# matteocarnelos/microflow-rs

Hardware: AMD Instinct MI355X
Metric: inferences/sec (int8) for person_detect.tflite (higher is better)
Workload: dtype i8; 1 GPU; person_detect.tflite batch=65536 per GPU, predict_inner int8->int8, inputs resident in HBM; per_gpu_batch=65536, global_batch=65536, parallelism=batch shard x1, no data-path collective

## Files before the change

### microflow_rs_amd/csrc/fused.hip

```cpp
#include <algorithm>
#include <cmath>
#include <cstdio>
#include <cstring>
#include <memory>

#include "ops_impl.hpp"
#include "wimage.hpp"

namespace mf {

struct FusedImpl {
    enum Kind { DWPW, TAIL, FCSM, STAGE, DWFC, PAIRTAIL, QUAD, CHAIN, FCCHAIN, POOLFC, PAIRBAND, PAIRWZ } kind;
    OpImpl *a, *b, *c;
    k::DwPwArgs dwpw;
    k::TailArgs tail;
    std::string name;
    k::StageArgs stage{};
    int stage_pairs = 0;
    std::vector<std::unique_ptr<DevBuf>> stage_w;
    k::DwFcArgs dwfc{};
    k::PairTailArgs pairtail{};
    k::PairFrontArgs pairfront{};
    bool has_front = false;
    k::QuadArgs quad{};
// ... 577 lines not shown
    if (magic != t.magic) return nullptr;
    std::unique_ptr<FusedImpl> f(new FusedImpl{FusedImpl::PAIRTAIL, dw, pairtail->b, pairtail->c, {}, {}, "pair_front_tail<6,6,128,2,256|3,3,256,2>"});
    f->pairtail = t, f->has_front = true, f->epi_mode = magic;
    k::PairFrontArgs &a = f->pairfront;
    a.dw_wmm = df.wmm, a.dwA = df.A, a.dwS = df.S, a.dwK = magic ? kc_with_magic(*f, dw->h_Kc) : df.Kc;
    a.dw_lo = df.lo_f, a.dw_hi = df.hi_f, a.izp4 = df.izp4;
    a.pw_w = plain_pw_image(*f, pw);
    a.pwA = pw->conv.A, a.pwS = pw->conv.S, a.pwK = magic ? kc_with_magic(*f, pw->h_Kc) : pw->conv.Kc;
    a.pw_lo = pw->conv.lo_f, a.pw_hi = pw->conv.hi_f;
    return f.release();
}

static FusedImpl *quad_group(FusedImpl *p1, FusedImpl *p2, const k::DwPwArgs &a, const k::DwPwArgs &b, const char *name, bool mm) {
    const OpSpec &d1 = p1->a->s, &q1 = p1->b->s, &d2 = p2->a->s, &q2 = p2->b->s;
    FusedImpl *f = new FusedImpl{FusedImpl::QUAD, p1->a, p2->b, nullptr, {}, {}, name};
    f->quad.a = a, f->quad.b = b, f->quad_mm = mm;
    f->epi_mode = std::min(pair_mode(a), pair_mode(b));
    f->quad_ops[0] = p1->a, f->quad_ops[1] = p1->b, f->quad_ops[2] = p2->a, f->quad_ops[3] = p2->b;
    const int shp[10] = {d1.H, d1.W, d1.C, d1.sh, q1.N, d2.H, d2.W, d2.C, d2.sh, q2.N};
    for (int i = 0; i < 10; ++i) f->quad_shape[i] = shp[i];
    return f;
}
FusedImpl *fused_quad_create(FusedImpl *p1, FusedImpl *p2) {
    const bool off = switches().no_quad;
    if (off || !p1 || !p2 || p1->kind != FusedImpl::DWPW || p2->kind != FusedImpl::DWPW) return nullptr;
    const OpSpec &d1 = p1->a->s, &q1 = p1->b->s, &d2 = p2->a->s, &q2 = p2->b->s;
    if (p1->a->device != p2->a->device || d1.u8 != d2.u8) return nullptr;
    if (d2.H != q1.H || d2.W != q1.W || d2.C != q1.N) return nullptr;
    if (k::quad_mm_shape(d1.H, d1.W, d1.C, d1.sh, q1.N, d2.H, d2.W, d2.C, d2.sh, q2.N)) {
        if (switches().no_quad_mm) return nullptr;
        k::DwPwArgs a = p1->dwpw, b = p2->dwpw;
        if (pair_mode(a) != 3 || pair_mode(b) != 3) a = pair_args(p1->a, p1->b, 0), b = pair_args(p2->a, p2->b, 0);
        if (!a.dw.wmm || !a.pw.wprep || !b.dw.wmm || !b.pw.wprep) return nullptr;
        if (!a.dw.magic || !a.pw.magic || !b.dw.magic || !b.pw.magic) return nullptr;
        return quad_group(p1, p2, a, b, "quad_mm<12,12,64,1,64|12,12,64,2,128>", true);
    }
    const char *nm = k::quad_name(d1.H, d1.W, d1.C, d1.sh, q1.N, d2.H, d2.W, d2.C, d2.sh, q2.N);
    if (!nm) return nullptr;
    const bool fma = p1->a->fma_strict() && p1->b->fma_strict() && p2->a->fma_strict() && p2->b->fma_strict();
    const k::DwPwArgs a = pair_args(p1->a, p1->b, fma ? 1 : 0), b = pair_args(p2->a, p2->b, fma ? 1 : 0);
    if (!a.dw.wmm || !a.pw.wrr || !b.dw.wmm || !b.pw.wrr) return nullptr;
    if (!a.dw.magic || !a.pw.magic || !b.dw.magic || !b.pw.magic) return nullptr;
    return quad_group(p1, p2, a, b, nm, false);
}

FusedImpl *fused_quad_stem_create(OpImpl *stem, FusedImpl *quad) {
    const bool off = switches().no_penta;
    if (off || !stem || !quad || quad->kind != FusedImpl::QUAD || quad->quad.stem || stem->fast != OpImpl::DW_STEM) return nullptr;
    const OpSpec &t = stem->s, &d1 = quad->a->s;
    if (stem->device != quad->a->device || t.u8 != d1.u8 || stem->force_generic) return nullptr;
    if (t.OH != d1.H || t.OW != d1.W || t.N != d1.C || t.sh != 2 || t.sw != 2 || t.C != 1) return nullptr;
    const int *q = quad->quad_shape;
    const char *nm = k::quad_stem_name(t.H, t.W, q[0], q[1], q[2], q[3], q[4], q[5], q[6], q[7], q[8], q[9]);
    if (!nm || !stem->stem.magic) return nullptr;
    std::unique_ptr<FusedImpl> f(new FusedImpl{FusedImpl::QUAD, stem, quad->b, nullptr, {}, {}, nm});
    f->quad = quad->quad;
    for (int i = 0; i < 10; ++i) f->quad_shape[i] = q[i];
    OpImpl *const *qo = quad->quad_ops;
    const bool fma = stem->fma_strict() && qo[0]->fma_strict() && qo[1]->fma_strict() && qo[2]->fma_strict() && qo[3]->fma_strict();
    f->quad.a = pair_args(qo[0], qo[1], fma ? 1 : 0), f->quad.b = pair_args(qo[2], qo[3], fma ? 1 : 0);
    k::DwStemArgs sa = stem->stem;
    if (fma) sa.use_fma();
    std::vector<uint32_t> tab(152);
    for (int l = 0; l < 64; ++l) tab[(size_t)2 * l] = sa.wmm[l][0], tab[(size_t)2 * l + 1] = sa.wmm[l][1];
    for (int c = 0; c < 8; ++c) {
        memcpy(&tab[(size_t)128 + c], &sa.A[c], 4);
// ... 414 lines not shown
```

### microflow_rs_amd/csrc/k_common.hpp

```cpp
#pragma once
#include <hip/hip_runtime.h>
#include <stdint.h>
#include <stdio.h>
#include <stdlib.h>

#include <atomic>
#include <type_traits>

#include "kernels.hpp"
#include "mf_switches.hpp"

namespace mf {
namespace k {

typedef int v4i __attribute__((ext_vector_type(4)));
typedef unsigned int u32x4 __attribute__((ext_vector_type(4)));

#ifndef MF_JITTER_DIAG
#define MF_JITTER_DIAG 0
#endif
__device__ __forceinline__ void mf_jitter() {
#if MF_JITTER_DIAG
    uint32_t t = (uint32_t)__builtin_readcyclecounter();
    t = (t ^ (t >> 7) ^ (threadIdx.x >> 6) * 0x9E3779B1u) * 0x85EBCA6Bu;
// ... 16 lines not shown
__device__ __forceinline__ int requant(int acc, float A, float S, float lo_f, float hi_f) {
    const float x = __fadd_rn(A, __fmul_rn(S, (float)acc));
    float r = __fadd_rn(x, __builtin_copysignf(0x1.fffffep-2f, x));
    r = __builtin_amdgcn_fmed3f(r, lo_f, hi_f);
    return (int)r;
}

template <int MG>
__device__ __forceinline__ int requant_t(int acc, float A, float S, float lo_f, float hi_f) {
    static_assert(MG != 3, "the single-fma form exists for the packed epilogues only (requant_pack4)");
    if constexpr (MG == 0) {
        return requant(acc, A, S, lo_f, hi_f);
    } else {
        const float f = __fsub_rn(__int_as_float(acc), 12582912.0f);
        const float x = __fadd_rn(A, __fmul_rn(S, f));
        float r = __fadd_rn(x, __builtin_copysignf(0x1.fffffep-2f, x));
        r = __builtin_amdgcn_fmed3f(r, lo_f, hi_f);
        return (int)r;
    }
}
template <int MG> __device__ __forceinline__ void epi_enter() {
    if constexpr (MG == 3) __builtin_amdgcn_s_setreg(0x801 , 3u );
}
#ifndef MF_EPI_PATCH_KO
#define MF_EPI_PATCH_KO 0
#endif
__device__ __forceinline__ EpiPatchRec epi_patch_load(const EpiPatchRec *tab, int idx) {
    typedef __attribute__((address_space(4))) const EpiPatchRec c_rec;
    if (MF_EPI_PATCH_KO || !tab) return EpiPatchRec{0, 0};
    c_rec *t = (c_rec *)(uintptr_t)tab;
    if (MF_EPI_PATCH_KO == 2) return EpiPatchRec{t[idx].P & 0, t[idx].meta};
    return EpiPatchRec{t[idx].P, t[idx].meta};
}
__device__ __forceinline__ void epi_patch_apply(v4i &a, const EpiPatchRec &rec, int g) {
    if (MF_EPI_PATCH_KO) return;
    if (__builtin_expect(rec.P != 0, 0)) {
        const bool any = (a[0] == rec.P) | (a[1] == rec.P) | (a[2] == rec.P) | (a[3] == rec.P);
        if (__builtin_expect(__builtin_amdgcn_ballot_w64(any) != 0ull, 0)) {
            asm volatile("" ::: "memory");
            const bool grp = g == ((rec.meta >> 2) & 3);
            const int delta = (rec.meta & 16) ? -1 : 1, reg = rec.meta & 3;
            a[0] += (grp && a[0] == rec.P) ? (reg == 0 ? delta : 0) : 0;
            a[1] += (grp && a[1] == rec.P) ? (reg == 1 ? delta : 0) : 0;
            a[2] += (grp && a[2] == rec.P) ? (reg == 2 ? delta : 0) : 0;
            a[3] += (grp && a[3] == rec.P) ? (reg == 3 ? delta : 0) : 0;
        }
    }
}
template <int MG> __device__ __forceinline__ int4 magic4(int4 k) {
    if constexpr (MG != 0) k.x += MF_MAGIC_I, k.y += MF_MAGIC_I, k.z += MF_MAGIC_I, k.w += MF_MAGIC_I;
    return k;
}

__device__ __forceinline__ int requant_any(int acc, float A, float S, float lo_f, float hi_f) {
    const float x = __fadd_rn(A, __fmul_rn(S, (float)acc));
    float r = __fadd_rn(x, __builtin_copysignf(0x1.fffffep-2f, x));
    r = (r != r) ? 0.0f : r;
    r = __builtin_amdgcn_fmed3f(r, lo_f, hi_f);
    return (int)r;
}

#ifndef MF_NT_STORE
#define MF_NT_STORE 0
#endif
template <bool NT> __device__ __forceinline__ void st_out_t(void *p, uint4 v) {
    if constexpr (NT) __builtin_nontemporal_store(v4i{(int)v.x, (int)v.y, (int)v.z, (int)v.w}, (v4i *)p);
    else *(v4i *)p = v4i{(int)v.x, (int)v.y, (int)v.z, (int)v.w};
}
template <bool NT> __device__ __forceinline__ void st_out_t(void *p, uint2 v) {
    typedef int v2i_ __attribute__((ext_vector_type(2)));
    if constexpr (NT) __builtin_nontemporal_store(v2i_{(int)v.x, (int)v.y}, (v2i_ *)p);
    else *(v2i_ *)p = v2i_{(int)v.x, (int)v.y};
}
template <bool NT> __device__ __forceinline__ void st_out_t(void *p, uint32_t v) {
    if constexpr (NT) __builtin_nontemporal_store(v, (uint32_t *)p);
    else *(uint32_t *)p = v;
}
template <typename V> __device__ __forceinline__ void st_out(void *p, V v) { st_out_t<MF_NT_STORE != 0>(p, v); }

__device__ __forceinline__ uint32_t pack4(int a, int b, int c, int d) {
// ... 264 lines not shown
        forced = now.dq_cfg;
        const char *l = now.dq_cfgs.c_str();
        if (*l) {
            int n = 1;
            for (const char *q = l; *q; ++q) n += *q == ',';
            int k = (int)(launches % (unsigned long)n);
            const char *q = l;
            while (k > 0 && *q) k -= *q++ == ',';
            forced = (int)strtol(q, nullptr, 0);
        }
    }
    if (forced) return forced;
    const double t_step = est_us * grid / (nsteps > 0 ? nsteps : 1);
    const int K = t_step >= 8.0 ? 1 : (t_step >= 4.0 ? 2 : 4);
    const double draws_per_us = nsteps / (K * (est_us > 1.0 ? est_us : 1.0));
    const double sfrac = sw.dq_static;
    int S0 = (int)(sfrac * (double)nsteps / (grid > 0 ? grid : 1));
    S0 = S0 < 2 ? 2 : (S0 > 32767 ? 32767 : S0);
    const int cfg = K | (draws_per_us > 60.0 ? 8 : 1) << 8 | S0 << 16;
    if (sw.dq_verbose) fprintf(stderr, "[microflow_amd] step queue: %d steps on %d workgroups, est %.0f us -> cfg 0x%x\n", nsteps, grid, est_us, cfg);
    return cfg;
}
static inline int *dq_slot(int *ring, unsigned long *launches) {
    if (!ring) return nullptr;
    const unsigned long n = launches ? __atomic_fetch_add(launches, 1ul, __ATOMIC_RELAXED) : dq_next_launch();
    return ring + (size_t)(n % (unsigned long)DYNQ_RING) * DynSteps::INTS;
}
static inline double dq_est_us(double hbm_bytes, double requant_bytes) {
    const double a = hbm_bytes / 4.5e6, b = requant_bytes / 4.0e6;
    return a > b ? a : b;
}

constexpr int cgcd(int a, int b) { return b == 0 ? a : cgcd(b, a % b); }
template <int TS> __device__ __forceinline__ constexpr int tile_swz(int x) {
    int r = 0;
    if constexpr ((TS & 0xf) != 0) r |= ((x >> ((TS & 0xf) - 1)) & 1);
    if constexpr (((TS >> 4) & 0xf) != 0) r |= ((x >> (((TS >> 4) & 0xf) - 1)) & 1) << 1;
    if constexpr (((TS >> 8) & 0xf) != 0) r |= ((x >> (((TS >> 8) & 0xf) - 1)) & 1) << 2;
    return r;
}

__device__ __forceinline__ float quant_div(float x, float scale, float rcp, bool fast) {
    if (!fast) return __fdiv_rn(x, scale);
    const float q0 = __fmul_rn(x, rcp);
    float q = __fmaf_rn(__fmaf_rn(-scale, q0, x), rcp, q0);
    if (!(__builtin_fabsf(q) <= 3.0e38f)) q = __fdiv_rn(x, scale);
    return q;
}

__device__ __forceinline__ void lane_group_transpose4(uint32_t &r0, uint32_t &r1, uint32_t &r2, uint32_t &r3) {
    typedef unsigned int u32x2 __attribute__((ext_vector_type(2)));
    u32x2 t;
    t = __builtin_amdgcn_permlane32_swap(r0, r2, false, false), r0 = t[0], r2 = t[1];
    t = __builtin_amdgcn_permlane32_swap(r1, r3, false, false), r1 = t[0], r3 = t[1];
    t = __builtin_amdgcn_permlane16_swap(r0, r1, false, false), r0 = t[0], r1 = t[1];
    t = __builtin_amdgcn_permlane16_swap(r2, r3, false, false), r2 = t[0], r3 = t[1];
}

struct LaunchState {
    static constexpr int MAX_DEV = 64;
    std::atomic<int> per_cu[MAX_DEV];
};
template <typename Kern> static int prepared(LaunchState &st, Kern kern, int threads, int lds_bytes) {
    int dev = 0;
    if (hipGetDevice(&dev) != hipSuccess || dev < 0 || dev >= LaunchState::MAX_DEV) dev = LaunchState::MAX_DEV - 1;
    int n = st.per_cu[dev].load(std::memory_order_relaxed);
// ... 40 lines not shown
```

### microflow_rs_amd/csrc/k_quad_mm.hip

```cpp
#include "k_common.hpp"

#ifndef MF_QMM_UB
#define MF_QMM_UB 2
#endif
#ifndef MF_QMM_KO
#define MF_QMM_KO 0
#endif
namespace mf {
namespace k {

namespace {
struct Q64 {
    static constexpr int G = 2, NTHR = 512, NWAVE = 8, NQ = 4, LP = 64, ROWB = 768;
    static constexpr int ROW_A = LP + ROWB + LP + 16, TILE_A = 14 * ROW_A, BUF_A = G * TILE_A;
    static constexpr int OPIX_A = 144, NPIX_A = G * OPIX_A, PLANE_A = NPIX_A * 16 + 16;
    static constexpr int ROW_B = LP + ROWB + LP, TILE_B = 14 * ROW_B, BUF_B = G * TILE_B, TS_B = 0x043;
    static constexpr int OPIX_B = 36, NPIX_B = G * OPIX_B, P16_B = 80, PLANE_B = P16_B * 16 + 16;
    static constexpr int OFF_TA = 0;
    static constexpr int OFF_MA = OFF_TA + BUF_A + 512;
    static constexpr int OFF_TB = OFF_MA + NQ * PLANE_A + 64;
    static constexpr int OFF_MB = OFF_TB + BUF_B + 512;
    static constexpr int OFF_C = OFF_MB + NQ * PLANE_B + 64;
    static constexpr int C_A_DW = 0, C_A_PW = 64 * 12, C_B_DW = 2 * 64 * 12, C_B_PW = 3 * 64 * 12, C_BYTES = 3 * 64 * 12 + 128 * 12;
    static constexpr int OFF_Q = OFF_C + C_BYTES;
    static constexpr int LDS = OFF_Q + 16;
};
static_assert(2 * Q64::LDS <= 160 * 1024, "two workgroups per CU");
static_assert(Q64::OFF_MA % 16 == 0 && Q64::OFF_TB % 16 == 0 && Q64::OFF_MB % 16 == 0, "16-byte aligned regions");
}

template <int MG, uint32_t XR4>
__global__ __launch_bounds__(512, 4) void quad_mm_12x12x64(const int8_t *__restrict__ in, int8_t *__restrict__ out, QuadArgs p, int batch) {
    using Z = Q64;
    constexpr int UB = MF_QMM_UB;
    epi_enter<MG>();
    extern __shared__ __attribute__((aligned(16))) uint8_t lds[];
    const int tid = threadIdx.x, lane = tid & 63;
    const int wave = __builtin_amdgcn_readfirstlane(tid >> 6);
    DynSteps dq;
    dq.init(lds + Z::OFF_Q, p.a.dw.queue, tid, p.a.dw.qcfg);

    for (int i = tid; i < (Z::BUF_A + 512) / 16; i += Z::NTHR)
        ((uint4 *)(lds + Z::OFF_TA))[i] = make_uint4(p.a.dw.izp4, p.a.dw.izp4, p.a.dw.izp4, p.a.dw.izp4);
    for (int i = tid; i < (Z::BUF_B + 512) / 16; i += Z::NTHR)
        ((uint4 *)(lds + Z::OFF_TB))[i] = make_uint4(p.b.dw.izp4, p.b.dw.izp4, p.b.dw.izp4, p.b.dw.izp4);

    const int col = lane & 15, g = lane >> 4;
    const int qa = wave & 3, ha = wave >> 2;
    const int cyA = col & 3, cxA = col >> 2;
    const int tbA = Z::OFF_TA + ha * Z::TILE_A + cyA * Z::ROW_A + Z::LP + (cxA + g - 1) * 64 + 16 * qa;
    const int mbA = Z::OFF_MA + qa * Z::PLANE_A + (ha * Z::OPIX_A + cyA * 12 + cxA) * 16 + 4 * g;
    const int cxB = col & 7, cyB = col >> 3;
    const int xlB = cxB * 2 + g - 1;
    const int tbB = Z::OFF_TB + ha * Z::TILE_B + cyB * 2 * Z::ROW_B + Z::LP + xlB * 64 + 16 * (qa ^ tile_swz<Z::TS_B>(xlB));
    const int mbB = Z::OFF_MB + qa * Z::PLANE_B + (ha * Z::OPIX_B + cyB * 6 + cxB) * 16 + 4 * g;
    const bool liveB = cxB < 6;
    v4i AdA[3], AdB[3];
#pragma unroll
    for (int ty = 0; ty < 3; ++ty) {
        AdA[ty] = ((const v4i *)p.a.dw.wmm)[(qa * 3 + ty) * 64 + lane];
        AdB[ty] = ((const v4i *)p.b.dw.wmm)[(qa * 3 + ty) * 64 + lane];
    }
    const v4i AwA = ((const v4i *)p.a.pw.wprep)[qa * 64 + lane];
    const int blk = wave >> 2, tt = wave & 3;
    const v4i AwB = ((const v4i *)p.b.pw.wprep)[wave * 64 + lane];
    {
        auto put = [&](int off, int n, const float *A, const float *S, const int *K) {
            for (int i = tid; i < n; i += Z::NTHR) {
                ((float *)(lds + Z::OFF_C + off))[i] = A[i], ((float *)(lds + Z::OFF_C + off))[n + i] = S[i];
                ((int *)(lds + Z::OFF_C + off))[2 * n + i] = K[i] + (MG != 0 ? MF_MAGIC_I : 0);
            }
        };
        put(Z::C_A_DW, 64, p.a.dw.A, p.a.dw.S, p.a.dw.Kc), put(Z::C_A_PW, 64, p.a.pw.A, p.a.pw.S, p.a.pw.Kc);
        put(Z::C_B_DW, 64, p.b.dw.A, p.b.dw.S, p.b.dw.Kc), put(Z::C_B_PW, 128, p.b.pw.A, p.b.pw.S, p.b.pw.Kc);
    }
    struct Consts {
        float4 a, s;
        int4 k;
    };
    auto consts = [&](int off, int n, int ch) {
        Consts c;
        c.a = *(const float4 *)(lds + Z::OFF_C + off + ch * 4), c.s = *(const float4 *)(lds + Z::OFF_C + off + (n + ch) * 4);
        c.k = *(const int4 *)(lds + Z::OFF_C + off + (2 * n + ch) * 4);
        return c;
    };
    const int ch_dw = 16 * qa + 4 * g, chA = g * 16 + 4 * qa, chB = blk * 64 + g * 16 + 4 * tt;
    int oB[9];
#pragma unroll
    for (int c = 0; c < 9; ++c) {
        const int pix = c * 16 + col, y = pix / 12, x = pix - y * 12;
        oB[c] = Z::OFF_TB + ha * Z::TILE_B + (y + 1) * Z::ROW_B + Z::LP + x * 64 + 16 * (g ^ tile_swz<Z::TS_B>(x)) + 4 * qa;
    }
    const EpiPatchRec prDA = epi_patch_load(MG == 3 ? p.a.dw.patch : nullptr, qa), prPA = epi_patch_load(MG == 3 ? p.a.pw.patch : nullptr, qa);
    const EpiPatchRec prDB = epi_patch_load(MG == 3 ? p.b.dw.patch : nullptr, qa), prPB = epi_patch_load(MG == 3 ? p.b.pw.patch : nullptr, wave);
    wg_sync();

    auto stage = [&](int st) {
#pragma unroll
        for (int k = 0; k < 3; ++k) {
            const int r = k * Z::NWAVE + wave, gi = r / 12, y = r % 12;
            if (st * Z::G + gi < batch && lane < 48)
                dma16(in + ((size_t)(st * Z::G + gi) * 9216 + y * Z::ROWB + lane * 16), lds + Z::OFF_TA + gi * Z::TILE_A + (y + 1) * Z::ROW_A + Z::LP);
        }
    };
    auto out_addr = [](int pix, int slot) { return Z::OFF_TB + (pix / 6 + 1) * Z::ROW_B + Z::LP + (pix % 6) * 128 + 16 * (slot ^ (pix & 7)); };
    auto copy_out = [&](int st, int gv) {
        int8_t *ob = out + (size_t)st * Z::G * Z::OPIX_B * 128;
        for (int j = tid; j < gv * Z::OPIX_B * 8; j += Z::NTHR) {
            const int pix = j >> 3, sp = j & 7;
            st_out(ob + pix * 128 + ((sp ^ (pix & 7)) << 4), *(const uint4 *)(lds + Z::OFF_TB + (pix / 6 + 1) * Z::ROW_B + Z::LP + (pix % 6) * 128 + sp * 16));
        }
    };

    const int nsteps = (batch + Z::G - 1) / Z::G;
    if (dq.step < nsteps) stage(dq.step);
    int prev = -1, prev_gv = 0;
    for (; dq.step < nsteps; dq.advance(tid)) {
        const int step = dq.step;
        asm volatile("s_waitcnt vmcnt(0)" ::: "memory");
        wg_sync();
        dq.top(tid);
        const int next = dq.nxt;
        const int gvalid = min(Z::G, batch - step * Z::G);
        if (prev >= 0 && !(MF_QMM_KO & 2)) copy_out(prev, prev_gv);

        {
            constexpr int NU = 9;
            const Consts k = consts(Z::C_A_DW, 64, ch_dw);
            auto toff = [](int t) constexpr { return (t / 3) * 4 * Z::ROW_A + (t % 3) * 4 * 64; };
            v4i bq[UB][3], bn[UB][3];
#pragma unroll
            for (int u = 0; u < UB; ++u)
#pragma unroll
                for (int ty = 0; ty < 3; ++ty) bq[u][ty] = *(const v4i *)(lds + tbA + toff(u < NU ? u : 0) + ty * Z::ROW_A);
#pragma unroll
            for (int t0 = 0; t0 < NU; t0 += UB) {
                v4i acc[UB];
#pragma unroll
                for (int u = 0; u < UB; ++u) acc[u] = v4i{k.k.x, k.k.y, k.k.z, k.k.w};
#pragma unroll
                for (int ty = 0; ty < 3; ++ty)
#pragma unroll
                    for (int u = 0; u < UB; ++u)
                        if (t0 + u < NU) acc[u] = __builtin_amdgcn_mfma_i32_16x16x64_i8(AdA[ty], bq[u][ty], acc[u], 0, 0, 0);
#pragma unroll
                for (int u = 0; u < UB; ++u)
                    if (t0 + UB + u < NU) {
#pragma unroll
                        for (int ty = 0; ty < 3; ++ty) bn[u][ty] = *(const v4i *)(lds + tbA + toff(t0 + UB + u) + ty * Z::ROW_A);
                    }
#pragma unroll
                for (int u = 0; u < UB; ++u)
                    if (t0 + u < NU) {
                        const int t = t0 + u;
                        if constexpr (MG == 3) epi_patch_apply(acc[u], prDA, g);
                        const uint32_t d = (MF_QMM_KO & 16) ? (uint32_t)(acc[u][0] ^ acc[u][1] ^ acc[u][2] ^ acc[u][3])
                                                            : requant_pack4<MG, XR4>(acc[u][0], acc[u][1], acc[u][2], acc[u][3], k.a, k.s, p.a.dw.lo_f, p.a.dw.hi_f);
                        *(uint32_t *)(lds + mbA + ((t / 3) * 4 * 12 + (t % 3) * 4) * 16) = d;
                    }
#pragma unroll
                for (int u = 0; u < UB; ++u)
#pragma unroll
                    for (int ty = 0; ty < 3; ++ty) bq[u][ty] = bn[u][ty];
            }
        }
        wg_sync();
        if (next < nsteps && !((MF_QMM_KO & 8) && prev >= 0)) stage((MF_QMM_KO & 32) ? (int)(blockIdx.x & 63) : next);

        {
            constexpr int NC = 9;
            const Consts k = consts(Z::C_A_PW, 64, chA);
            const uint8_t *mid = lds + Z::OFF_MA + g * Z::PLANE_A + (ha * Z::OPIX_A + col) * 16;
            v4i bq[UB], bn[UB];
#pragma unroll
            for (int u = 0; u < UB; ++u) bq[u] = *(const v4i *)(mid + (u < NC ? u : 0) * 256);
#pragma unroll
            for (int c0 = 0; c0 < NC; c0 += UB) {
                v4i acc[UB];
#pragma unroll
                for (int u = 0; u < UB; ++u)
                    if (c0 + u < NC) acc[u] = __builtin_amdgcn_mfma_i32_16x16x64_i8(AwA, bq[u], v4i{k.k.x, k.k.y, k.k.z, k.k.w}, 0, 0, 0);
#pragma unroll
                for (int u = 0; u < UB; ++u)
                    if (c0 + UB + u < NC) bn[u] = *(const v4i *)(mid + (c0 + UB + u) * 256);
#pragma unroll
                for (int u = 0; u < UB; ++u)
                    if (c0 + u < NC) {
                        if constexpr (MG == 3) epi_patch_apply(acc[u], prPA, g);
                        const uint32_t d = (MF_QMM_KO & 16) ? (uint32_t)(acc[u][0] ^ acc[u][1] ^ acc[u][2] ^ acc[u][3])
                                                            : requant_pack4<MG, XR4>(acc[u][0], acc[u][1], acc[u][2], acc[u][3], k.a, k.s, p.a.pw.lo_f, p.a.pw.hi_f);
                        *(uint32_t *)(lds + oB[c0 + u]) = d;
                    }
#pragma unroll
                for (int u = 0; u < UB; ++u) bq[u] = bn[u];
            }
        }
        if (!(MF_QMM_KO & 1)) wg_sync();

        if (!(MF_QMM_KO & 4)) {
            constexpr int NU = 3;
            const Consts k = consts(Z::C_B_DW, 64, ch_dw);
            v4i bq[NU][3];
#pragma unroll
            for (int t = 0; t < NU; ++t)
#pragma unroll
// ... 74 lines not shown
```

### microflow_rs_amd/csrc/kernels.hpp

```cpp
#pragma once
#include <hip/hip_runtime.h>
#include <stddef.h>
#include <stdint.h>

#include <vector>

namespace mf {
namespace k {

extern thread_local unsigned long long launches_enqueued;
#define MF_LAUNCH(...)                      \
    do {                                    \
        ++::mf::k::launches_enqueued;       \
        hipLaunchKernelGGL(__VA_ARGS__);    \
    } while (0)

struct F32Edge {
    float in_scale, in_rcp, in_zp_f, in_sat_lo, in_sat_hi;
    uint32_t in_xr4;
    int in_fast;
    float out_scale, out_zp_f;
};
constexpr int EDGE_IN = 1, EDGE_OUT = 2;

// ... 34 lines not shown
    const float *A;
    const int *Kc;
    const int *rowsum;
    int *rs_sums;
    int *rs_sync;
    int wzp;
    float S;
    float lo_f, hi_f;
    int M, N, K;
    uint32_t xr4;
};
struct SoftmaxArgs {
    int rows, cols;
    float oscale, ozp_f;
    const float *exp_table;
    float sat_lo, sat_hi;
    int xr;
};
constexpr int MF_MAGIC_I = 0x4B400000;
constexpr int EPI_PATCH_MAX = 4;
struct EpiPatch {
    int n;
    int ch[EPI_PATCH_MAX];
    int P[EPI_PATCH_MAX];
    int R[EPI_PATCH_MAX];
};
struct EpiPatchRec {
    int P;
    int meta;
};
static inline EpiPatchRec epi_patch_rec(int P, int R, int reg, int lane_group) {
    return EpiPatchRec{P, (reg & 3) | (lane_group & 3) << 2 | (R < P ? 16 : 0)};
}
constexpr int DYNQ_INTS = 8 * 32 + 32;
constexpr int DYNQ_RING = 32;
struct DwFastArgs {
    const int8_t *w;
    const void *wmm;
    const void *wsp;
    const void *wblk;
    const float *A;
    const float *S;
    const int *Kc;
    uint32_t izp4;
    float lo_f, hi_f;
    int magic;
    int xr;
    int *queue;
    unsigned long *qlaunch;
    int qcfg;
    const float *A3, *S3;
    const int *Kc3;
    int npatch3;
    const EpiPatchRec *patch;
    bool use_fma(bool with_patches = false) {
        if (!A3 || (npatch3 != 0 && !with_patches)) return false;
        return A = A3, S = S3, Kc = Kc3, magic = 3, true;
    }
};
struct DwC1Args {
    int H, W, N, KH, KW, sh, sw, OH, OW, pad_same;
    int izp;
    float lo_f, hi_f;
    int KG, TWP;
    const uint32_t *wpack;
    const float *A;
    const float *S;
    const int *Kc;
    int magic, xr;
};
struct DwStemArgs {
    uint32_t wrow[3][8];
    uint32_t wmm[64][2];
// ... 566 lines not shown
```

### microflow_rs_amd/csrc/ops.hip

```cpp
#include <algorithm>
#include <array>
#include <cmath>
#include <cstdio>
#include <cstdlib>
#include <cstring>
#include <map>
#include <memory>
#include <mutex>

#include "ops_impl.hpp"
#include "wimage.hpp"

namespace mf {

int dev_count() {
    int n = 0;
    if (hipGetDeviceCount(&n) != hipSuccess) {
        (void)hipGetLastError();
        return 0;
    }
    return n;
}

void dev_require(int device) {
// ... 196 lines not shown
}
template <typename F> void epi_fields_izp(F &f, const OpImpl &op, const ConvCtx &c) {
    f.izp4 = 0x01010101u * (uint32_t)(uint8_t)(int8_t)c.s.izp;
    epi_fields(f, op, c);
}
template <typename F> void step_queue(F &f, OpImpl &op) { f.queue = (int *)op.d_queue.p, f.qlaunch = &op.q_launches; }

struct ConstPtrs {
    const float *A, *S;
    const int *Kc, *wzp;
};
ConstPtrs channel_consts(const OpImpl &op) { return {op.conv.A, op.conv.S, op.conv.Kc, op.conv.wzp}; }
template <typename M> ConstPtrs row_consts(OpImpl &op, const ConvCtx &c, size_t np, int rows, M ch_of) {
    std::vector<float> pA(np, 0.0f), pS(np, 0.0f);
    std::vector<int32_t> pK(np, 0), pZ(np, 0);
    for (int r = 0; r < rows; ++r) {
        const size_t ch = (size_t)ch_of(r);
        pA[(size_t)r] = c.A[ch], pS[(size_t)r] = c.S[ch], pK[(size_t)r] = c.Kc[ch], pZ[(size_t)r] = c.wzp[ch];
    }
    op.d_rtA.upload(pA.data(), np * 4), op.d_rtS.upload(pS.data(), np * 4);
    op.d_rtKc.upload(pK.data(), np * 4), op.d_rtwzp.upload(pZ.data(), np * 4);
    return {op.d_rtA.as<float>(), op.d_rtS.as<float>(), op.d_rtKc.as<int>(), op.d_rtwzp.as<int>()};
}


bool route_dw_table(OpImpl &op, const ConvCtx &c) {
    const OpSpec &s = c.s;
    if (!(!switches().no_table && c.dw && c.zero_wzp && c.same3x3 && s.C == s.N && k::dw_fast_name(s.H, s.W, s.C, s.sh))) return false;
    op.fast = OpImpl::DW_NHWC;
    op.fast_name = k::dw_fast_name(s.H, s.W, s.C, s.sh);
    k::DwFastArgs &f = op.dwf;
    f.w = op.conv.w, f.A = op.conv.A, f.S = op.conv.S, f.Kc = op.conv.Kc;
    epi_fields_izp(f, op, c);
    f.wmm = nullptr, f.wsp = nullptr, f.wblk = nullptr;
    step_queue(f, op);
    if (s.C == 8 || s.C % 16 == 0) {
        const std::vector<int8_t> prep = wimage::build_dw_mm_weights(s.weights, s.C);
        op.d_wprep.upload(prep.data(), prep.size());
        f.wmm = op.d_wprep.p;
        const std::vector<int8_t> sp = wimage::build_dw_sp_weights(prep, s.C == 8 ? 1 : s.C / 16);
        if (!sp.empty()) {
            op.d_wsp.upload(sp.data(), sp.size());
            f.wsp = op.d_wsp.p;
        }
        if (s.sh == 1) {
            const std::vector<int8_t> blk = wimage::build_dw_blk_weights(s.weights, s.C);
            op.d_wblk.upload(blk.data(), blk.size());
            f.wblk = op.d_wblk.p;
        }
        if (dw_taps_on_matrix_pipe() && k::dw_mm_name(s.H, s.W, s.C, s.sh)) op.fast_name = k::dw_mm_name(s.H, s.W, s.C, s.sh);
    }
    return true;
}

bool route_dw_stem(OpImpl &op, const ConvCtx &c) {
    const OpSpec &s = c.s;
    if (!(!switches().no_table && c.dw && c.zero_wzp && c.same3x3 && s.C == 1 && k::dw_stem_name(s.H, s.W, s.N, s.sh))) return false;
    op.fast = OpImpl::DW_STEM;
    op.fast_name = k::dw_stem_name(s.H, s.W, s.N, s.sh);
    k::DwStemArgs &f = op.stem;
    step_queue(f, op);
    wimage::build_stem_rows(s.weights, s.N, f.wrow);
    wimage::build_stem_mm(s.weights, s.N, &f.wmm[0][0], 2);
    for (int ch = 0; ch < 8; ++ch) f.A[ch] = c.A[ch], f.S[ch] = c.S[ch], f.Kc[ch] = c.Kc[ch];
    epi_fields_izp(f, op, c);
    return true;
}

bool route_dw_stem_rt(OpImpl &op, const ConvCtx &c) {
    const OpSpec &s = c.s;
    if (!(!switches().no_rt && !switches().no_stem_rt && c.dw && c.zero_wzp && c.same3x3 && s.C == 1 && s.sh == 2 &&
          k::dw_stem_rt_plan(op.stemrt, s.H, s.W, s.N, s.OH, s.OW)))
        return false;
    op.fast = OpImpl::DW_STEM_RT;
    op.fast_name = "dw3x3_stem_rt<" + std::to_string(s.N) + ">";
    k::DwStemRtArgs &f = op.stemrt;
    step_queue(f, op);
    wimage::build_stem_mm(s.weights, s.N, &f.wmm[0][0], 4);
    for (int ch = 0; ch < 8; ++ch) f.A[ch] = c.A[(size_t)(ch % s.N)], f.S[ch] = c.S[(size_t)(ch % s.N)], f.Kc[ch] = c.Kc[(size_t)(ch % s.N)];
    epi_fields_izp(f, op, c);
    return true;
// ... 786 lines not shown
```

### microflow_rs_amd/csrc/ops_impl.hpp

```cpp
#pragma once
#include <hip/hip_runtime.h>

#include <cstdint>
#include <string>
#include <vector>

#include "kernels.hpp"
#include "mf_internal.hpp"

namespace mf {

#define MF_HIP(call)                                                                          \
    do {                                                                                      \
        hipError_t e_ = (call);                                                               \
        if (e_ != hipSuccess)                                                                 \
            fail(e_ == hipErrorOutOfMemory ? MF_ERR_OOM : MF_ERR_HIP,                         \
                 std::string(#call) + ": " + hipGetErrorString(e_));                          \
    } while (0)

inline int32_t wrap_add(int32_t a, int32_t b) { return (int32_t)((uint32_t)a + (uint32_t)b); }
inline int32_t wrap_sub(int32_t a, int32_t b) { return (int32_t)((uint32_t)a - (uint32_t)b); }
inline int32_t wrap_mul(int32_t a, int32_t b) { return (int32_t)((uint32_t)a * (uint32_t)b); }

struct DevBuf {
// ... 35 lines not shown
    bool finite_consts = true;
    std::string generic_name, fast_name;
    enum Fast { NONE, DW_NHWC, DW_STEM, DW_STEM_RT, DW_C1, PW_MFMA, FC_ROWWAVE, FC_MFMA, POOL_C4, CONV1X1_ROW, DW_RT, PW_RT, CONV_ROWS, CONV_MM, FC_RT,
                CONV_GEMM, DW_GEMM, FC_SPARSE24 } fast = NONE;
    int *d_rowsum = nullptr;
    size_t rowsum_cap = 0, rowsum_rows = 0;
    int8_t *d_ext = nullptr;
    size_t ext_cap = 0;
    hipEvent_t scratch_ev = nullptr;
    bool scratch_used = false;
    static bool capturing(hipStream_t s) {
        hipStreamCaptureStatus st = hipStreamCaptureStatusNone;
        if (hipStreamIsCapturing(s, &st) != hipSuccess) (void)hipGetLastError();
        return st != hipStreamCaptureStatusNone;
    }
    void scratch_acquire(hipStream_t s, bool growing) {
        if (capturing(s)) {
            if (growing) fail(MF_ERR_HIP, "a scratch buffer would have to grow inside a stream capture");
            return;
        }
        if (!scratch_ev) MF_HIP(hipEventCreateWithFlags(&scratch_ev, hipEventDisableTiming));
        if (scratch_used) {
            if (growing) MF_HIP(hipEventSynchronize(scratch_ev));
            else MF_HIP(hipStreamWaitEvent(s, scratch_ev, 0));
        }
    }
    void scratch_release(hipStream_t s) {
        if (capturing(s)) return;
        if (!scratch_ev) MF_HIP(hipEventCreateWithFlags(&scratch_ev, hipEventDisableTiming));
        MF_HIP(hipEventRecord(scratch_ev, s));
        scratch_used = true;
    }

    DevBuf d_w, d_wzp, d_A, d_S, d_Kc, d_wprep, d_wsp, d_wblk, d_wrr, d_wiso, d_table;
    std::vector<int8_t> h_w;
    std::vector<float> h_A, h_S;
    std::vector<int32_t> h_Kc, h_wzp;
    std::vector<uint32_t> h_wpack;
    unsigned long q_launches = 0;
    DevBuf d_queue;
    k::DwC1Args dwc1{};
    k::ConvArgs conv{};
    k::PoolArgs pool{};
    k::FcArgs fc{};
    k::SoftmaxArgs sm{};
    k::DwFastArgs dwf{};
    k::DwStemArgs stem{};
    k::DwStemRtArgs stemrt{};
    k::PwArgs pw{};
    k::DwRtArgs dwrt{};
    k::PwRtArgs pwrt{};
    k::FcRtArgs fcrt{};
    bool fcrt_ok = false;
    DevBuf d_fcw, d_fcA, d_fcKc;
    DevBuf d_sp24;
    k::ConvRowsArgs crows{};
    k::ConvMmArgs cmm{};
    DevBuf d_tap;
    k::ConvGemmArgs cgm{};
    DevBuf d_cgm_mask;
    k::DwGemmArgs dwg{};
    DevBuf d_crw, d_crm;
    bool rt_wz = false;
    int magic_mode = 0;
    bool fma_ok = false;
    k::EpiPatch fma_patch{};
    bool fma_strict() const { return fma_ok && fma_patch.n == 0; }
// ... 9 lines not shown
```

### microflow_rs_amd/csrc/wimage.cpp

```cpp
#include "wimage.hpp"

#include <cstring>

namespace mf {
namespace wimage {

std::vector<int8_t> build_pw_weights(const int8_t *w , int K, int N) {
    const int NB = N < 64 ? N : 64, TB = NB / 16, NSPLIT = N / NB;
    const int KS = K < 64 ? 1 : K / 64, Q = K < 64 ? 64 / K : 1;
    std::vector<int8_t> out((size_t)NSPLIT * Q * TB * KS * 64 * 16, 0);
    for (int blk = 0; blk < NSPLIT; ++blk)
        for (int q = 0; q < Q; ++q)
            for (int tt = 0; tt < TB; ++tt)
                for (int ks = 0; ks < KS; ++ks)
                    for (int lane = 0; lane < 64; ++lane) {
                        const int r = lane & 15, g = lane >> 4;
                        const int gr = r >> 2, j = r & 3;
                        const int ch = blk * NB + gr * (NB / 4) + 4 * tt + j;
                        int8_t *dst = &out[(((((size_t)blk * Q + q) * TB + tt) * KS + ks) * 64 + lane) * 16];
                        for (int i = 0; i < 16; ++i) {
                            int k = -1;
                            if (K >= 64) k = ks * 64 + g * 16 + i;
                            else if (K == 32) k = ((g >> 1) == q) ? (g & 1) * 16 + i : -1;
                            else if (K == 16) k = (g == q) ? i : -1;
// ... 42 lines not shown
                    for (int b = 0; b < 4; ++b)
                        if (blk[4 * grp + b] != 0) pos[n++] = b;
                    if (n > 2) return {};
                    if (n == 0) pos[0] = 0, pos[1] = 1;
                    if (n == 1) pos[1] = (pos[0] + 1) & 3;
                    for (int j = 0; j < 2; ++j) {
                        const int sb = 8 * ha + 2 * grp + j;
                        dst[sb] = j < n ? blk[4 * grp + pos[j]] : (int8_t)0;
                        idx |= (uint32_t)pos[j] << (2 * sb);
                    }
                }
            }
            memcpy(dst + 16, &idx, 4);
            if (ga < 2) memcpy(dst + 20, block(q, 2, 2, r) + 8 * ga, 8);
        }
    return out;
}

std::vector<int8_t> build_dw_blk_weights(const int8_t *w , int C) {
    const int NQ4 = C / 4;
    std::vector<int8_t> out((size_t)NQ4 * 64 * 16, 0);
    for (int q = 0; q < NQ4; ++q)
        for (int lane = 0; lane < 64; ++lane) {
            const int m = lane & 15, g = lane >> 4, s = m >> 2, i = m & 3, ty = g - (s >> 1);
            if (ty < 0 || ty > 2) continue;
            for (int xx = 0; xx < 4; ++xx) {
                const int tx = xx - (s & 1);
                if (tx >= 0 && tx <= 2) out[((size_t)q * 64 + lane) * 16 + 4 * xx + i] = w[(ty * 3 + tx) * C + 4 * q + i];
            }
        }
    return out;
}

std::vector<int8_t> build_pw_iso_weights(const int8_t *w , int N) {
    const int NT = N / 16;
    std::vector<int8_t> out((size_t)4 * NT * 64 * 8, 0);
    for (int s = 0; s < 4; ++s)
        for (int t = 0; t < NT; ++t)
            for (int m = 0; m < 16; ++m)
                memcpy(&out[(((size_t)s * NT + t) * 64 + 16 * s + m) * 8], w + (size_t)(16 * t + m) * 8, 8);
    return out;
}

std::vector<int8_t> build_dw_mm_rt_weights(const int8_t *w, int KH, int KW, int C, int KS ,
                                           int P) {
    const int NQ = (C + 15) / 16, T = KH * KW;
    std::vector<int8_t> out((size_t)NQ * KS * 1024, 0);
    for (int q = 0; q < NQ; ++q)
        for (int ks = 0; ks < KS; ++ks)
            for (int lane = 0; lane < 64; ++lane) {
                const int r = lane & 15, t = 4 * ks + (lane >> 4);
                const int c = P > 1 ? (r < P * C ? r % C : -1) : (16 * q + r < C ? 16 * q + r : -1);
                if (t < T && c >= 0) out[(((size_t)q * KS + ks) * 64 + lane) * 16 + r] = w[(size_t)t * C + c];
            }
    return out;
}

std::vector<int8_t> build_dw_mm_weights_sp(const int8_t *w , int C, int S) {
    const int P = 16 / C;
    std::vector<int8_t> out((size_t)3 * 64 * 16, 0);
    for (int ty = 0; ty < 3; ++ty)
        for (int lane = 0; lane < 64; ++lane) {
            const int r = lane & 15, g = lane >> 4, p = r / C, c = r % C;
            int8_t *dst = &out[((size_t)ty * 64 + lane) * 16];
            for (int pp = 0; pp < P; ++pp) {
                const int tx = P * (g - 1) + pp - S * p + 1;
// ... 142 lines not shown
```

### microflow_rs_amd/csrc/wimage.hpp

```cpp
#pragma once
#include <cstddef>
#include <cstdint>
#include <vector>

namespace mf {
namespace wimage {

std::vector<int8_t> build_pw_weights(const int8_t *w , int K, int N);
std::vector<int8_t> build_dw_mm_weights(const int8_t *w , int C);
std::vector<int8_t> build_dw_sp_weights(const std::vector<int8_t> &dense , int NQ);
std::vector<int8_t> build_dw_blk_weights(const int8_t *w , int C);
std::vector<int8_t> build_pw_iso_weights(const int8_t *w , int N);
std::vector<int8_t> build_dw_mm_rt_weights(const int8_t *w, int KH, int KW, int C, int KS ,
                                           int P = 1);
std::vector<int8_t> build_dw_mm_weights_sp(const int8_t *w , int C, int S);
std::vector<int8_t> build_pw_rr_weights(const int8_t *w , int K, int N);
std::vector<int8_t> build_pw_rt_weights(const int8_t *w , int K, int N, int group, bool ones);
std::vector<int8_t> build_pw_rt_reg_weights(const int8_t *w , int K, int N, int group, int TB, int NBLK);
std::vector<int8_t> build_pw_plain_weights(const int8_t *w, int K, int N);

void fill_ones_tile(int8_t *dst , int K, int KS);
std::vector<int8_t> build_dw_ones_image();
std::vector<int8_t> build_pw_ones_tile(int C);
void build_stem_rows(const int8_t *w , int N, uint32_t wrow[3][8]);
void build_stem_mm(const int8_t *w , int N, uint32_t *wmm , int pitch);
std::vector<uint32_t> build_conv_rows_pack(const int8_t *w, bool depthwise, int KH, int KW, int C, int N, int KG, int NP);
inline std::vector<uint32_t> build_dw_c1_pack(const int8_t *w , int KH, int KW, int N, int KG) { return build_conv_rows_pack(w, true, KH, KW, 1, N, KG, 8); }
std::vector<uint32_t> build_conv_rows_mask(int RWB , int KG);

}
}
```

Baseline: 30.96 million inferences/s.

## Pack two output rows per MFMA in quad_mm depthwise stage A

Adds a two-row depthwise layout for the first depthwise conv in the quad_mm kernel. Each MFMA now covers two output rows with an 8-channel octet per wave, using 2 weight fragments instead of 3 and 64-bit LDS reads with immediate offsets. The LDS tile and mid-plane pitches are padded to odd 8-byte strides to avoid bank conflicts, and the unroll depth rises from 2 to 3. The aim is fewer MFMA instructions and LDS reads per tap, at the cost of a new weight image, reworked epilogue-patch lane mapping and more register pressure.

```diff
diff --git a/microflow_rs_amd/csrc/fused.hip b/microflow_rs_amd/csrc/fused.hip
--- a/microflow_rs_amd/csrc/fused.hip
+++ b/microflow_rs_amd/csrc/fused.hip
@@ -633,6 +633,7 @@
         k::DwPwArgs a = p1->dwpw, b = p2->dwpw;
         if (pair_mode(a) != 3 || pair_mode(b) != 3) a = pair_args(p1->a, p1->b, 0), b = pair_args(p2->a, p2->b, 0);
         if (!a.dw.wmm || !a.pw.wprep || !b.dw.wmm || !b.pw.wprep) return nullptr;
+        if (MF_DW_TWOROW && !a.dw.wtr) return nullptr;
         if (!a.dw.magic || !a.pw.magic || !b.dw.magic || !b.pw.magic) return nullptr;
         return quad_group(p1, p2, a, b, "quad_mm<12,12,64,1,64|12,12,64,2,128>", true);
     }
diff --git a/microflow_rs_amd/csrc/k_common.hpp b/microflow_rs_amd/csrc/k_common.hpp
--- a/microflow_rs_amd/csrc/k_common.hpp
+++ b/microflow_rs_amd/csrc/k_common.hpp
@@ -72,13 +72,13 @@
     if (MF_EPI_PATCH_KO == 2) return EpiPatchRec{t[idx].P & 0, t[idx].meta};
     return EpiPatchRec{t[idx].P, t[idx].meta};
 }
-__device__ __forceinline__ void epi_patch_apply(v4i &a, const EpiPatchRec &rec, int g) {
+template <typename F> __device__ __forceinline__ void epi_patch_apply_if(v4i &a, const EpiPatchRec &rec, F lanes) {
     if (MF_EPI_PATCH_KO) return;
     if (__builtin_expect(rec.P != 0, 0)) {
         const bool any = (a[0] == rec.P) | (a[1] == rec.P) | (a[2] == rec.P) | (a[3] == rec.P);
         if (__builtin_expect(__builtin_amdgcn_ballot_w64(any) != 0ull, 0)) {
             asm volatile("" ::: "memory");
-            const bool grp = g == ((rec.meta >> 2) & 3);
+            const bool grp = lanes();
             const int delta = (rec.meta & 16) ? -1 : 1, reg = rec.meta & 3;
             a[0] += (grp && a[0] == rec.P) ? (reg == 0 ? delta : 0) : 0;
             a[1] += (grp && a[1] == rec.P) ? (reg == 1 ? delta : 0) : 0;
@@ -86,6 +86,9 @@
             a[3] += (grp && a[3] == rec.P) ? (reg == 3 ? delta : 0) : 0;
         }
     }
+}
+__device__ __forceinline__ void epi_patch_apply(v4i &a, const EpiPatchRec &rec, int g) {
+    epi_patch_apply_if(a, rec, [&] { return g == ((rec.meta >> 2) & 3); });
 }
 template <int MG> __device__ __forceinline__ int4 magic4(int4 k) {
     if constexpr (MG != 0) k.x += MF_MAGIC_I, k.y += MF_MAGIC_I, k.z += MF_MAGIC_I, k.w += MF_MAGIC_I;
@@ -416,6 +419,20 @@
 }
 
 constexpr int cgcd(int a, int b) { return b == 0 ? a : cgcd(b, a % b); }
+typedef int v2i __attribute__((ext_vector_type(2)));
+template <int OFF> __device__ __forceinline__ v2i lds_read8(int lds_byte_addr) {
+    static_assert(OFF >= 0 && OFF < 65536, "16-bit instruction offset");
+    v2i r;
+    asm volatile("ds_read_b64 %0, %1 offset:%2" : "=v"(r) : "v"(lds_byte_addr), "n"(OFF));
+    return r;
+}
+template <int N, typename F> __device__ __forceinline__ void static_for(F &&f) {
+    if constexpr (N > 0) {
+        static_for<N - 1>(f);
+        f(std::integral_constant<int, N - 1>{});
+    }
+}
+
 template <int TS> __device__ __forceinline__ constexpr int tile_swz(int x) {
     int r = 0;
     if constexpr ((TS & 0xf) != 0) r |= ((x >> ((TS & 0xf) - 1)) & 1);
diff --git a/microflow_rs_amd/csrc/k_quad_mm.hip b/microflow_rs_amd/csrc/k_quad_mm.hip
--- a/microflow_rs_amd/csrc/k_quad_mm.hip
+++ b/microflow_rs_amd/csrc/k_quad_mm.hip
@@ -1,7 +1,8 @@
 #include "k_common.hpp"
+#include "wimage.hpp"
 
 #ifndef MF_QMM_UB
-#define MF_QMM_UB 2
+#define MF_QMM_UB (MF_DW_TWOROW ? 3 : 2)
 #endif
 #ifndef MF_QMM_KO
 #define MF_QMM_KO 0
@@ -12,8 +13,14 @@
 namespace {
 struct Q64 {
     static constexpr int G = 2, NTHR = 512, NWAVE = 8, NQ = 4, LP = 64, ROWB = 768;
+#if MF_DW_TWOROW
+    static constexpr int ROW_A = LP + ROWB + LP + 8, TILE_A = 14 * ROW_A + 8, BUF_A = G * TILE_A;
+    static constexpr int OPIX_A = 144, MIMG_A = OPIX_A + 4, NPIX_A = G * MIMG_A, PLANE_A = NPIX_A * 16 + 128;
+    static_assert((ROW_A / 8) % 2 == 1 && (TILE_A / 8) % 2 == 1 && BUF_A % 16 == 0, "odd 8-byte pitches");
+#else
     static constexpr int ROW_A = LP + ROWB + LP + 16, TILE_A = 14 * ROW_A, BUF_A = G * TILE_A;
-    static constexpr int OPIX_A = 144, NPIX_A = G * OPIX_A, PLANE_A = NPIX_A * 16 + 16;
+    static constexpr int OPIX_A = 144, MIMG_A = OPIX_A, NPIX_A = G * OPIX_A, PLANE_A = NPIX_A * 16 + 16;
+#endif
     static constexpr int ROW_B = LP + ROWB + LP, TILE_B = 14 * ROW_B, BUF_B = G * TILE_B, TS_B = 0x043;
     static constexpr int OPIX_B = 36, NPIX_B = G * OPIX_B, P16_B = 80, PLANE_B = P16_B * 16 + 16;
     static constexpr int OFF_TA = 0;
@@ -47,20 +54,38 @@
 
     const int col = lane & 15, g = lane >> 4;
     const int qa = wave & 3, ha = wave >> 2;
+#if MF_DW_TWOROW
+    auto tapA = [&](int img, int yp, int x) { return Z::OFF_TA + img * Z::TILE_A + (2 * yp + (g >> 1)) * Z::ROW_A + Z::LP + (x - 1 + 2 * (g & 1)) * 64 + 8 * wave; };
+    auto midA = [&](int img, int yp, int x) {
+        return Z::OFF_MA + (wave >> 1) * Z::PLANE_A + (img * Z::MIMG_A + (2 * yp + (g >> 1)) * 12 + x) * 16 + 8 * (wave & 1) + 4 * (g & 1);
+    };
+    const int tbA1 = tapA((col >> 2) & 1, col & 3, col >> 3), mbA1 = midA((col >> 2) & 1, col & 3, col >> 3);
+    const int tbA2 = tapA((col >> 1) & 1, 4 + (col & 1), col >> 2), mbA2 = midA((col >> 1) & 1, 4 + (col & 1), col >> 2);
+    const int tbA1b = tbA1 + 64, tbA2b = tbA2 + 64;
+#else
     const int cyA = col & 3, cxA = col >> 2;
     const int tbA = Z::OFF_TA + ha * Z::TILE_A + cyA * Z::ROW_A + Z::LP + (cxA + g - 1) * 64 + 16 * qa;
     const int mbA = Z::OFF_MA + qa * Z::PLANE_A + (ha * Z::OPIX_A + cyA * 12 + cxA) * 16 + 4 * g;
+#endif
     const int cxB = col & 7, cyB = col >> 3;
     const int xlB = cxB * 2 + g - 1;
     const int tbB = Z::OFF_TB + ha * Z::TILE_B + cyB * 2 * Z::ROW_B + Z::LP + xlB * 64 + 16 * (qa ^ tile_swz<Z::TS_B>(xlB));
     const int mbB = Z::OFF_MB + qa * Z::PLANE_B + (ha * Z::OPIX_B + cyB * 6 + cxB) * 16 + 4 * g;
     const bool liveB = cxB < 6;
+#if MF_DW_TWOROW
+    v4i AdA[2], AdB[3];
+#pragma unroll
+    for (int j = 0; j < 2; ++j) AdA[j] = ((const v4i *)p.a.dw.wtr)[(wave * 2 + j) * 64 + lane];
+#pragma unroll
+    for (int ty = 0; ty < 3; ++ty) AdB[ty] = ((const v4i *)p.b.dw.wmm)[(qa * 3 + ty) * 64 + lane];
+#else
     v4i AdA[3], AdB[3];
 #pragma unroll
     for (int ty = 0; ty < 3; ++ty) {
         AdA[ty] = ((const v4i *)p.a.dw.wmm)[(qa * 3 + ty) * 64 + lane];
         AdB[ty] = ((const v4i *)p.b.dw.wmm)[(qa * 3 + ty) * 64 + lane];
     }
+#endif
     const v4i AwA = ((const v4i *)p.a.pw.wprep)[qa * 64 + lane];
     const int blk = wave >> 2, tt = wave & 3;
     const v4i AwB = ((const v4i *)p.b.pw.wprep)[wave * 64 + lane];
@@ -91,7 +116,14 @@
         const int pix = c * 16 + col, y = pix / 12, x = pix - y * 12;
         oB[c] = Z::OFF_TB + ha * Z::TILE_B + (y + 1) * Z::ROW_B + Z::LP + x * 64 + 16 * (g ^ tile_swz<Z::TS_B>(x)) + 4 * qa;
     }
+#if MF_DW_TWOROW
+    EpiPatchRec prDA = epi_patch_load(MG == 3 ? p.a.dw.patch : nullptr, wave >> 1);
+    if (!wimage::dw_tworow_patch_octet(prDA.meta, wave)) prDA.P = 0;
+    const EpiPatchRec prPA = epi_patch_load(MG == 3 ? p.a.pw.patch : nullptr, qa);
+    const int ch_dwA = 8 * wave + 4 * (g & 1);
+#else
     const EpiPatchRec prDA = epi_patch_load(MG == 3 ? p.a.dw.patch : nullptr, qa), prPA = epi_patch_load(MG == 3 ? p.a.pw.patch : nullptr, qa);
+#endif
     const EpiPatchRec prDB = epi_patch_load(MG == 3 ? p.b.dw.patch : nullptr, qa), prPB = epi_patch_load(MG == 3 ? p.b.pw.patch : nullptr, wave);
     wg_sync();
 
@@ -124,6 +156,51 @@
         const int gvalid = min(Z::G, batch - step * Z::G);
         if (prev >= 0 && !(MF_QMM_KO & 2)) copy_out(prev, prev_gv);
 
+#if MF_DW_TWOROW
+        {
+            constexpr int NU = 9, NB = (NU + UB - 1) / UB;
+            const Consts k = consts(Z::C_A_DW, 64, ch_dwA);
+            auto taps = [&](auto U, v4i(&b)[2]) {
+                constexpr int u = decltype(U)::value, o = u < 6 ? u * 2 * 64 : (u - 6) * 4 * 64;
+                const int a0 = u < 6 ? tbA1 : tbA2, a1 = u < 6 ? tbA1b : tbA2b;
+                const v2i l0 = lds_read8<o>(a0), h0 = lds_read8<o>(a1), l1 = lds_read8<o + 2 * Z::ROW_A>(a0), h1 = lds_read8<o + 2 * Z::ROW_A>(a1);
+                b[0] = v4i{l0.x, l0.y, h0.x, h0.y}, b[1] = v4i{l1.x, l1.y, h1.x, h1.y};
+            };
+            auto tap_wait = [](v4i(&b)[2]) { asm volatile("s_waitcnt lgkmcnt(0)" : "+v"(b[0]), "+v"(b[1])); };
+            v4i bq[UB][2], bn[UB][2];
+            static_for<UB>([&](auto U) { taps(std::integral_constant<int, (U.value < NU ? U.value : 0)>{}, bq[U.value]); });
+            static_for<NB>([&](auto T) {
+                constexpr int t0 = decltype(T)::value * UB;
+                v4i acc[UB];
+#pragma unroll
+                for (int u = 0; u < UB; ++u) acc[u] = v4i{k.k.x, k.k.y, k.k.z, k.k.w};
+#pragma unroll
+                for (int u = 0; u < UB; ++u) tap_wait(bq[u]);
+#pragma unroll
+                for (int j = 0; j < 2; ++j)
+#pragma unroll
+                    for (int u = 0; u < UB; ++u)
+                        if (t0 + u < NU) acc[u] = __builtin_amdgcn_mfma_i32_16x16x64_i8(AdA[j], bq[u][j], acc[u], 0, 0, 0);
+                static_for<UB>([&](auto U) {
+                    constexpr int u = decltype(U)::value;
+                    if constexpr (t0 + UB + u < NU) taps(std::integral_constant<int, t0 + UB + u>{}, bn[u]);
+                });
+#pragma unroll
+                for (int u = 0; u < UB; ++u)
+                    if (t0 + u < NU) {
+                        const int t = t0 + u;
+                        if constexpr (MG == 3) epi_patch_apply_if(acc[u], prDA, [&] { return wimage::dw_tworow_patch_lane(prDA.meta, g); });
+                        const uint32_t d = (MF_QMM_KO & 16) ? (uint32_t)(acc[u][0] ^ acc[u][1] ^ acc[u][2] ^ acc[u][3])
+                                                            : requant_pack4<MG, XR4>(acc[u][0], acc[u][1], acc[u][2], acc[u][3], k.a, k.s, p.a.dw.lo_f, p.a.dw.hi_f);
+                        *(uint32_t *)(lds + (t < 6 ? mbA1 + t * 2 * 16 : mbA2 + (t - 6) * 4 * 16)) = d;
+                    }
+#pragma unroll
+                for (int u = 0; u < UB; ++u)
+#pragma unroll
+                    for (int j = 0; j < 2; ++j) bq[u][j] = bn[u][j];
+            });
+        }
+#else
         {
             constexpr int NU = 9;
             const Consts k = consts(Z::C_A_DW, 64, ch_dw);
@@ -164,13 +241,14 @@
                     for (int ty = 0; ty < 3; ++ty) bq[u][ty] = bn[u][ty];
             }
         }
+#endif
         wg_sync();
         if (next < nsteps && !((MF_QMM_KO & 8) && prev >= 0)) stage((MF_QMM_KO & 32) ? (int)(blockIdx.x & 63) : next);
 
         {
             constexpr int NC = 9;
             const Consts k = consts(Z::C_A_PW, 64, chA);
-            const uint8_t *mid = lds + Z::OFF_MA + g * Z::PLANE_A + (ha * Z::OPIX_A + col) * 16;
+            const uint8_t *mid = lds + Z::OFF_MA + g * Z::PLANE_A + (ha * Z::MIMG_A + col) * 16;
             v4i bq[UB], bn[UB];
 #pragma unroll
             for (int u = 0; u < UB; ++u) bq[u] = *(const v4i *)(mid + (u < NC ? u : 0) * 256);
diff --git a/microflow_rs_amd/csrc/kernels.hpp b/microflow_rs_amd/csrc/kernels.hpp
--- a/microflow_rs_amd/csrc/kernels.hpp
+++ b/microflow_rs_amd/csrc/kernels.hpp
@@ -90,6 +90,9 @@
 static inline EpiPatchRec epi_patch_rec(int P, int R, int reg, int lane_group) {
     return EpiPatchRec{P, (reg & 3) | (lane_group & 3) << 2 | (R < P ? 16 : 0)};
 }
+#ifndef MF_DW_TWOROW
+#define MF_DW_TWOROW 1
+#endif
 constexpr int DYNQ_INTS = 8 * 32 + 32;
 constexpr int DYNQ_RING = 32;
 struct DwFastArgs {
@@ -97,6 +100,7 @@
     const void *wmm;
     const void *wsp;
     const void *wblk;
+    const void *wtr;
     const float *A;
     const float *S;
     const int *Kc;
diff --git a/microflow_rs_amd/csrc/ops.hip b/microflow_rs_amd/csrc/ops.hip
--- a/microflow_rs_amd/csrc/ops.hip
+++ b/microflow_rs_amd/csrc/ops.hip
@@ -252,7 +252,7 @@
     k::DwFastArgs &f = op.dwf;
     f.w = op.conv.w, f.A = op.conv.A, f.S = op.conv.S, f.Kc = op.conv.Kc;
     epi_fields_izp(f, op, c);
-    f.wmm = nullptr, f.wsp = nullptr, f.wblk = nullptr;
+    f.wmm = nullptr, f.wsp = nullptr, f.wblk = nullptr, f.wtr = nullptr;
     step_queue(f, op);
     if (s.C == 8 || s.C % 16 == 0) {
         const std::vector<int8_t> prep = wimage::build_dw_mm_weights(s.weights, s.C);
@@ -267,6 +267,9 @@
             const std::vector<int8_t> blk = wimage::build_dw_blk_weights(s.weights, s.C);
             op.d_wblk.upload(blk.data(), blk.size());
             f.wblk = op.d_wblk.p;
+            const std::vector<int8_t> tr = wimage::build_dw_tworow_weights(s.weights, s.C);
+            op.d_wtr.upload(tr.data(), tr.size());
+            f.wtr = op.d_wtr.p;
         }
         if (dw_taps_on_matrix_pipe() && k::dw_mm_name(s.H, s.W, s.C, s.sh)) op.fast_name = k::dw_mm_name(s.H, s.W, s.C, s.sh);
     }
diff --git a/microflow_rs_amd/csrc/ops_impl.hpp b/microflow_rs_amd/csrc/ops_impl.hpp
--- a/microflow_rs_amd/csrc/ops_impl.hpp
+++ b/microflow_rs_amd/csrc/ops_impl.hpp
@@ -91,7 +91,7 @@
         scratch_used = true;
     }
 
-    DevBuf d_w, d_wzp, d_A, d_S, d_Kc, d_wprep, d_wsp, d_wblk, d_wrr, d_wiso, d_table;
+    DevBuf d_w, d_wzp, d_A, d_S, d_Kc, d_wprep, d_wsp, d_wblk, d_wtr, d_wrr, d_wiso, d_table;
     std::vector<int8_t> h_w;
     std::vector<float> h_A, h_S;
     std::vector<int32_t> h_Kc, h_wzp;
diff --git a/microflow_rs_amd/csrc/wimage.cpp b/microflow_rs_amd/csrc/wimage.cpp
--- a/microflow_rs_amd/csrc/wimage.cpp
+++ b/microflow_rs_amd/csrc/wimage.cpp
@@ -98,6 +98,22 @@
     return out;
 }
 
+std::vector<int8_t> build_dw_tworow_weights(const int8_t *w , int C) {
+    const int NO = C / 8;
+    std::vector<int8_t> out((size_t)NO * 2 * 64 * 16, 0);
+    for (int o = 0; o < NO; ++o)
+        for (int j = 0; j < 2; ++j)
+            for (int lane = 0; lane < 64; ++lane) {
+                const int m = lane & 15, g = lane >> 4, r = m >> 3, c = m & 7, ty = 2 * j + (g >> 1) - r;
+                if (ty < 0 || ty > 2) continue;
+                for (int pp = 0; pp < 2; ++pp) {
+                    const int tx = 2 * (g & 1) + pp;
+                    if (tx <= 2) out[(((size_t)o * 2 + j) * 64 + lane) * 16 + 8 * pp + c] = w[(ty * 3 + tx) * C + 8 * o + c];
+                }
+            }
+    return out;
+}
+
 std::vector<int8_t> build_pw_iso_weights(const int8_t *w , int N) {
     const int NT = N / 16;
     std::vector<int8_t> out((size_t)4 * NT * 64 * 8, 0);
diff --git a/microflow_rs_amd/csrc/wimage.hpp b/microflow_rs_amd/csrc/wimage.hpp
--- a/microflow_rs_amd/csrc/wimage.hpp
+++ b/microflow_rs_amd/csrc/wimage.hpp
@@ -10,6 +10,9 @@
 std::vector<int8_t> build_dw_mm_weights(const int8_t *w , int C);
 std::vector<int8_t> build_dw_sp_weights(const std::vector<int8_t> &dense , int NQ);
 std::vector<int8_t> build_dw_blk_weights(const int8_t *w , int C);
+std::vector<int8_t> build_dw_tworow_weights(const int8_t *w , int C);
+constexpr bool dw_tworow_patch_octet(int meta, int octet) { return ((meta >> 3) & 1) == (octet & 1); }
+constexpr bool dw_tworow_patch_lane(int meta, int g) { return (g & 1) == ((meta >> 2) & 1); }
 std::vector<int8_t> build_pw_iso_weights(const int8_t *w , int N);
 std::vector<int8_t> build_dw_mm_rt_weights(const int8_t *w, int KH, int KW, int C, int KS ,
                                            int P = 1);
```

Result: no change. 31.12 million inferences/s, median of 6 (+0.5%).
